# jh-jeong/ContraD

Hardware: AMD Instinct MI355X
Metric: discriminator-step images/sec (ContraD, SimCLR aug) (higher is better)
Workload: dtype f32; 1 GPU; SNDCGAN + ContraD D-step, CIFAR-10 32x32, global batch 512, simclr aug, nonsat loss, Adam(2e-4,(0.5,0.999)), random-init weights; global_batch=512, per_gpu_batch=512, parallelism=dp1, losses_finite=True, launch=hipGraph replay, rccl_ranks=1

## Files before the change

### contrad_amd/_lib.py

```python
import ctypes
import os
import re

_HERE = os.path.dirname(os.path.abspath(__file__))
LIB_PATH = os.environ.get('CONTRAD_HIP_LIB') or os.path.join(_HERE, 'csrc', 'libcontrad_hip.so')
HEADER_PATH = os.path.join(os.path.dirname(_HERE), 'include', 'contrad_hip.h')


class ConvDesc(ctypes.Structure):
    _fields_ = [(n, ctypes.c_int) for n in
                ('N', 'H', 'W', 'C', 'ldx', 'Ho', 'Wo', 'K', 'ldy', 'KH', 'KW', 'stride', 'pad', 'ldw')]


SN_MAX_LAYERS = 24
ADAM_MAX_TENSORS = 64
ADAM_CHUNK = 16384
AUG_NPARAM = 16


class SnLayer(ctypes.Structure):
    _fields_ = [('w', ctypes.c_void_p), ('u', ctypes.c_void_p), ('v', ctypes.c_void_p),
                ('u_snap', ctypes.c_void_p), ('v_snap', ctypes.c_void_p),
                ('wp', ctypes.c_void_p), ('gwp', ctypes.c_void_p), ('gw', ctypes.c_void_p),
                ('K', ctypes.c_int), ('C', ctypes.c_int), ('T', ctypes.c_int), ('ldw', ctypes.c_int),
# ... 43 lines not shown
                ('rowloss', ctypes.c_void_p), ('loss', ctypes.c_void_p), ('grad_scale', ctypes.c_void_p),
                ('dz', ctypes.c_void_p), ('workspace', ctypes.c_void_p), ('workspace_bytes', ctypes.c_longlong)]


class L2normProblem(ctypes.Structure):
    _fields_ = [('u', ctypes.c_void_p), ('z', ctypes.c_void_p), ('inv_norm', ctypes.c_void_p), ('dz', ctypes.c_void_p),
                ('du', ctypes.c_void_p), ('ldu', ctypes.c_int), ('R', ctypes.c_int), ('D', ctypes.c_int),
                ('accumulate', ctypes.c_int), ('zero_rows', ctypes.c_int)]


FILTER_MAX_JOBS = 16


class FilterJob(ctypes.Structure):
    _fields_ = [('wp', ctypes.c_void_p), ('U', ctypes.c_void_p), ('kind', ctypes.c_int), ('mode', ctypes.c_int),
                ('C', ctypes.c_int), ('K', ctypes.c_int), ('ldw', ctypes.c_int)]


class FilterBatch(ctypes.Structure):
    _fields_ = [('n', ctypes.c_int), ('jobs', FilterJob * FILTER_MAX_JOBS),
                ('block_start', ctypes.c_int * (FILTER_MAX_JOBS + 1))]


_CTYPES = {
    'int': ctypes.c_int,
    'float': ctypes.c_float,
    'double': ctypes.c_double,
    'long long': ctypes.c_longlong,
    'contrad_stream_t': ctypes.c_void_p,
    'void': None,
}


def _map_type(t):
    t = t.strip()
    if t.endswith('*'):
        base = t[:-1].replace('const', '').strip()
        if base == 'contrad_conv_desc':
            return ctypes.POINTER(ConvDesc)
        if base == 'int':
            return ctypes.POINTER(ctypes.c_int)
        return ctypes.c_void_p
    t = t.replace('const', '').strip()
    return _CTYPES[t]


# ... 48 lines not shown
```

### contrad_amd/csrc/igemm.hip

```cpp
#include "common.h"
#include <stdlib.h>
#include <string.h>
#include <algorithm>
#include <utility>
#include "../../include/contrad_hip.h"

namespace {

enum { MODE_FWD = 0, MODE_DGRAD = 1, MODE_WGRAD = 2 };
#ifndef IGEMM_BK
#define IGEMM_BK 16
#endif
constexpr int BK = IGEMM_BK;
#ifndef IGEMM_MIN_WAVES
#define IGEMM_MIN_WAVES 4
#endif
constexpr int NTHREADS = 256;

struct IgemmArgs {
  const float* A;
  const float* B;
  float* C;
  const float* bias;
  const float* addend;
  const float* act_ref;
  float* bias_ws;
  contrad_conv_desc d;
  float slope, gain;
  int M, Ncol, Kg;
  int tiles_m, tiles_n;
  int P;
  int ptiles_per_split;
  int ny;
  int cgroup;
  int cbal;
  int cb_reps[4], cb_start[5];
  int dsplits;
  long long slab_elems;
  int px_pixels;
  short win_h0[16], win_w0[16], win_hc[16], win_wc[16];
  int win_tile0[17];
  int nwin;
  unsigned char px_order[256];
  int pixmajor;
  int px_full;
  int st_nt;
};

constexpr long long NT_STORE_BYTES = 256ll << 20;
inline int st_nt_for(long long rows, int ld) {
#if defined(LEAN_ST_NT)
  if (LEAN_ST_NT >= 0) return LEAN_ST_NT;
#endif
  return rows * (long long)ld * (long long)sizeof(float) >= NT_STORE_BYTES ? 1 : 0;
}

__device__ __forceinline__ float4 ld4(const float* p) { return *reinterpret_cast<const float4*>(p); }
__device__ __forceinline__ float4 zero4() { return make_float4(0.f, 0.f, 0.f, 0.f); }

template <int MODE, int BM, int BN, bool VEC>
__global__ __launch_bounds__(NTHREADS, 2) void igemm_kernel(const IgemmArgs p) {
  extern __shared__ __attribute__((aligned(16))) float smem[];
  constexpr bool A_KCONTIG = (MODE != MODE_WGRAD);
  constexpr bool B_KCONTIG = (MODE == MODE_DGRAD);
  constexpr int LDA = BM + (A_KCONTIG ? 1 : 4);
  constexpr int LDB = BN + (B_KCONTIG ? 1 : 4);
  constexpr int A_SZ = BK * LDA, B_SZ = BK * LDB;
  constexpr int PA = BM * BK / 1024, PB = BN * BK / 1024;
  constexpr int KQ = BK / 4;
// ... 526 lines not shown
            p.C[off + c] = v;
          }
        }
      }
  } else {
#pragma unroll
    for (int i = 0; i < TM; ++i)
#pragma unroll
      for (int r = 0; r < 16; ++r) {
        const int m = m0 + wm * WM + i * 32 + (r & 3) + 8 * (r >> 2) + 4 * lhi;
        if (m >= M) continue;
#pragma unroll
        for (int j = 0; j < TN; ++j) {
          const int c = n0 + wn * WN + j * 32 + l31;
          if (c < Ncol) {
            float v = acc[i][j][r];
            if constexpr (MODE == MODE_FWD) {
              if (p.bias) v += p.bias[c];
              v = (v > 0.f) ? v : v * p.slope;
              v *= p.gain;
              if (p.addend) v += p.addend[(size_t)m * d.ldy + c];
              p.C[(size_t)m * d.ldy + c] = v;
            } else {
              p.C[((size_t)blockIdx.y * M + m) * Ncol + c] = v;
            }
          }
        }
      }
    if constexpr (MODE == MODE_WGRAD && VEC) {
      if (p.bias_ws != nullptr && tile_m == 0) {
        float* red = smem;
        *reinterpret_cast<float4*>(red + b_r * BN + b_c4 * 4) = colacc;
        __syncthreads();
        if (tid < BN) {
          float sum = 0.f;
#pragma unroll
          for (int r = 0; r < B_RPP; ++r) sum += red[r * BN + tid];
          const int c = n0 + tid;
          if (c < Ncol) p.bias_ws[(size_t)blockIdx.y * Ncol + c] = sum;
        }
      }
    }
  }
}

__global__ void wgrad_reduce_kernel(const float* __restrict__ ws, float* __restrict__ out, int Kg, int Ncol,
                                    int ldw, int splits, const float* __restrict__ bias_ws,
                                    float* __restrict__ dbias, int R) {
  const long long total = (long long)Kg * Ncol;
  const long long nthreads = (long long)gridDim.x * blockDim.x;
  const long long t0 = (long long)blockIdx.x * blockDim.x + threadIdx.x;
  const int r = (int)(t0 % R);
  const long long g0 = t0 / R, gstride = nthreads / R;
  if (ldw == Ncol && (total & 3) == 0) {
    const long long n4 = total / 4;
    for (long long q0 = g0 - (g0 % (64 / R)); q0 < n4; q0 += gstride) {
      const long long q = q0 + (g0 % (64 / R));
      float4 s = make_float4(0.f, 0.f, 0.f, 0.f);
      if (q < n4) {
        int k = r;
        for (; k + 3 * R < splits; k += 4 * R) {
          const float4 v0 = *reinterpret_cast<const float4*>(ws + (long long)k * total + q * 4);
          const float4 v1 = *reinterpret_cast<const float4*>(ws + (long long)(k + R) * total + q * 4);
          const float4 v2 = *reinterpret_cast<const float4*>(ws + (long long)(k + 2 * R) * total + q * 4);
          const float4 v3 = *reinterpret_cast<const float4*>(ws + (long long)(k + 3 * R) * total + q * 4);
          s.x += (v0.x + v1.x) + (v2.x + v3.x); s.y += (v0.y + v1.y) + (v2.y + v3.y);
          s.z += (v0.z + v1.z) + (v2.z + v3.z); s.w += (v0.w + v1.w) + (v2.w + v3.w);
        }
        for (; k < splits; k += R) {
          const float4 v = *reinterpret_cast<const float4*>(ws + (long long)k * total + q * 4);
          s.x += v.x; s.y += v.y; s.z += v.z; s.w += v.w;
        }
      }
      for (int o = R >> 1; o > 0; o >>= 1) {
// ... 6 lines not shown
    for (long long e0 = g0 - (g0 % (64 / R)); e0 < total; e0 += gstride) {
      const long long e = e0 + (g0 % (64 / R));
      float s = 0.f;
      if (e < total)
        for (int k = r; k < splits; k += R) s += ws[(long long)k * total + e];
      for (int o = R >> 1; o > 0; o >>= 1) s += __shfl_xor(s, o, 64);
      if (r == 0 && e < total) {
        const int i = (int)(e / Ncol), c = (int)(e - (long long)i * Ncol);
        out[(size_t)i * ldw + c] = s;
      }
    }
  }
  if (dbias)
    for (long long c0 = g0 - (g0 % (64 / R)); c0 < Ncol; c0 += gstride) {
      const long long c = c0 + (g0 % (64 / R));
      float s = 0.f;
      if (c < Ncol)
        for (int k = r; k < splits; k += R) s += bias_ws[(long long)k * Ncol + c];
      for (int o = R >> 1; o > 0; o >>= 1) s += __shfl_xor(s, o, 64);
      if (r == 0 && c < Ncol) dbias[c] = s;
    }
}

template <int BM, int BN>
constexpr size_t smem_bytes(int mode) {
  const int lda = BM + ((mode != MODE_WGRAD) ? 1 : 4);
  const int ldb = BN + ((mode == MODE_DGRAD) ? 1 : 4);
  size_t main_loop = 2 * (size_t)(BK * lda + BK * ldb) * sizeof(float);
  size_t epi = (size_t)BM * sizeof(long long);
  return main_loop > epi ? main_loop : epi;
}

template <auto Kernel, class Args>
int launch_large_lds(dim3 grid, int threads, size_t lds_bytes, hipStream_t stream, const Args& a) {
  static bool attr_set_dev[64] = {};
  int dev_id = 0;
  (void)hipGetDevice(&dev_id);
  bool& attr_set = attr_set_dev[dev_id & 63];
  if (!attr_set) {
    hipError_t e = hipFuncSetAttribute(reinterpret_cast<const void*>(Kernel), hipFuncAttributeMaxDynamicSharedMemorySize, (int)lds_bytes);
    if (e != hipSuccess) return (int)e;
    attr_set = true;
  }
  hipLaunchKernelGGL(Kernel, grid, dim3(threads), lds_bytes, stream, a);
  CONTRAD_CHECK_LAUNCH();
  return 0;
// ... 612 lines not shown
                                    int ldx, const float* __restrict__ act_ref, float slope, float gain,
                                    float* __restrict__ dx) {
  const int c4n = C >> 2;
  const long long total = rows * c4n;
  const float g1 = gain, g0 = gain * slope;
  for (long long e = (long long)blockIdx.x * blockDim.x + threadIdx.x; e < total;
       e += (long long)gridDim.x * blockDim.x) {
    const long long m = e / c4n;
    const long long off = m * ldx + (e - m * c4n) * 4;
    float4 v = ld4(ws + off);
    for (int k = 1; k < splits; ++k) {
      const float4 u = ld4(ws + (long long)k * slab + off);
      v.x += u.x; v.y += u.y; v.z += u.z; v.w += u.w;
    }
    if (act_ref) {
      const float4 a = ld4(act_ref + off);
      v.x *= (a.x > 0.f) ? g1 : g0; v.y *= (a.y > 0.f) ? g1 : g0;
      v.z *= (a.z > 0.f) ? g1 : g0; v.w *= (a.w > 0.f) ? g1 : g0;
    }
    *reinterpret_cast<float4*>(dx + off) = v;
  }
}

int launch_wgrad_reduce(const float* ws, float* dwp, int Kg, int K, int ldw, int slabs, const float* bias_ws, float* dbias,
                        hipStream_t stream) {
  const long long total = (long long)Kg * K;
  int R = 1;
  while (R < 64 && R * 2 <= slabs && (total / 4) * R < 65536) R <<= 1;
  const long long blocks = std::max(1ll, std::min(2048ll, ((total / 4) * R + 255) / 256));
  hipLaunchKernelGGL(wgrad_reduce_kernel, dim3((int)blocks), dim3(256), 0, stream, ws, dwp, Kg, K, ldw, slabs, bias_ws, dbias, R);
  CONTRAD_CHECK_LAUNCH();
  return 0;
}

template <int MODE>
int launch_wino_kind(int kind, const contrad_conv_desc* d, const float* in, const float* wp, const float* bias, const float* ref,
                     float* out, float slope, float gain, float* workspace, const contrad_filter_job* u, hipStream_t stream) {
  CONTRAD_ARG(aligned16(in, wp, workspace));
  const float* U = filter_fits(u, kind, MODE, d, wp) ? u->U : nullptr;
  const WinoFamily* f = wino_family(kind);
  CONTRAD_ARG(f && f->launch[MODE]);
  return f->launch[MODE](d, in, wp, bias, ref, out, slope, gain, workspace, stream, U);
}

enum Family {
  FAM_SCALAR = 0, FAM_GENERAL = 1, FAM_LEAN = 2, FAM_LEAN_SKIP = 3,
  FAM_WGRAD_C32 = 4, FAM_FWD_K1 = 5, FAM_CONV_C32 = 6,
  FAM_WINO = 7, FAM_WINO22 = 8, FAM_WINO44 = 9, FAM_WINO23 = 10, FAM_WINO44N = 11
};

inline const WinoFamily* wino_family_of(int family) { return wino_family(family == FAM_WINO44N ? FILTER_WINO44 : family); }

struct Route {
  int family;
  int filter_kind;
// ... 397 lines not shown
  const dim3 grid = mode == MODE_FWD ? fwd_setup(d, r.plan, &a) : mode == MODE_DGRAD ? dgrad_setup(d, r.plan, &a) : wgrad_setup(d, r.plan, &a);
  if (mode == MODE_FWD && !with_workspace) return grid.x;
  return (long long)grid.x * grid.y;
}

extern "C" int contrad_conv2d_tile_order(const contrad_conv_desc* d, int mode, unsigned char* out, int capacity) {
  if (check_desc(d) || (mode != MODE_FWD && mode != MODE_DGRAD) || !out || capacity <= 0) return -22;
  const Route r = conv_route(d, mode, true, 0);
  if (r.family != FAM_LEAN_SKIP || r.plan.pixmajor != 1 || r.plan.splits > 1) return 0;
  const int npix = mode == MODE_FWD ? d->Ho * d->Wo : cdiv(d->H, d->stride) * cdiv(d->W, d->stride);
  unsigned char order[256] = {};
  if (!pixel_table(d, mode, r.plan, npix, order)) return 0;
  const int nt = cdiv(d->N, r.plan.bm) * npix;
  if (nt > capacity) return -22;
  memcpy(out, order, (size_t)nt);
  return nt;
}

extern "C" long long contrad_conv2d_wgrad_workspace_bytes(const contrad_conv_desc* d) {
  if (check_desc(d)) return -22;
  return conv_route(d, MODE_WGRAD, true).workspace_bytes;
}

extern "C" int contrad_conv2d_wgrad(const contrad_conv_desc* d, const float* x, const float* gy,
                                    float* dwp, float* dbias, float* workspace, long long workspace_bytes,
                                    contrad_stream_t stream) {
  int rc = check_desc(d);
  if (rc) return rc;
  CONTRAD_ARG(x && gy && dwp && workspace);
  if (vec_ok(d, MODE_WGRAD)) CONTRAD_ARG(aligned16(x, gy, workspace));
  const Route r = conv_route(d, MODE_WGRAD, true);
  CONTRAD_ARG(workspace_bytes >= r.workspace_bytes);
  hipStream_t s = (hipStream_t)stream;
  const int Kg = d->KH * d->KW * d->C;
  switch (r.family) {
    case FAM_WINO: return launch_wgrad<WinoWgrad>(d, x, gy, dwp, dbias, workspace, s);
    case FAM_WINO22: return launch_wgrad<Wino22Wgrad>(d, x, gy, dwp, dbias, workspace, s);
    case FAM_WGRAD_C32: {
      const int blocks = wgrad_c32_blocks(d);
      float* bias_ws = dbias ? workspace + (size_t)blocks * Kg * d->K : nullptr;
      rc = launch_wgrad_c32(d, x, gy, workspace, bias_ws, s);
      return rc ? rc : launch_wgrad_reduce(workspace, dwp, Kg, d->K, d->ldw, blocks, bias_ws, dbias, s);
    }
    default: break;
  }
  const FwdPlan& p = r.plan;
  CONTRAD_ARG(dbias == nullptr || r.vec);
  CONTRAD_ARG((long long)d->N * d->Ho * d->Wo < (1ll << 31) - 4096);
  IgemmArgs a{};
  a.A = x; a.B = gy; a.C = workspace;
  a.bias_ws = dbias ? workspace + (size_t)p.splits * Kg * d->K : nullptr;
  const dim3 grid = wgrad_setup(d, p, &a);
  rc = dispatch<MODE_WGRAD>(a, p.bm, p.bn, r.vec, grid, s);
  return rc ? rc : launch_wgrad_reduce(workspace, dwp, Kg, d->K, d->ldw, p.splits, a.bias_ws, dbias, s);
}
```

### contrad_amd/csrc/igemm_lean.h

```cpp
#pragma once

#ifndef LEAN_DEEP
#define LEAN_DEEP 0
#endif
#ifndef LEAN_LD_NT
#define LEAN_LD_NT 0
#endif
#ifndef LEAN_ST_NT
#define LEAN_ST_NT -1
#endif
#ifndef LEAN_QPAD
#define LEAN_QPAD 8
#endif

constexpr unsigned LEAN_OOB = 0x80000000u;
constexpr unsigned LEAN_RANGE = 0x80000000u;
constexpr unsigned WB_TOP = 2u, WB_BOT = 4u, WB_LEFT = 8u, WB_RIGHT = 16u;

__device__ __forceinline__ float4 bload4(__amdgpu_buffer_rsrc_t r, unsigned voff, unsigned soff) {
  return __builtin_bit_cast(float4, __builtin_amdgcn_raw_buffer_load_b128(r, (int)voff, (int)soff, 0));
}

__device__ __forceinline__ __amdgpu_buffer_rsrc_t lean_rsrc(const float* base, bool on) {
  return __builtin_amdgcn_make_buffer_rsrc(const_cast<float*>(base), 0, on ? (int)LEAN_RANGE : 0, 0x00020000);
// ... 640 lines not shown
#pragma unroll
        for (int q = 0; q < EPI_G; ++q) {
#pragma unroll
          for (int jj = 0; jj < TN; ++jj) {
            const unsigned vo = offs[q] + colpart[jj];
            float v = acc[i][jj][r0 + q];
            if constexpr (MODE == MODE_DGRAD) {
              if (ref) v *= (rv[q][jj] > 0.f) ? g1 : g0;
            } else {
              v += bj[jj];
              v = (v > 0.f) ? v : v * p.slope;
              v *= p.gain;
              if (ref) v += rv[q][jj];
            }
            __builtin_amdgcn_raw_buffer_store_b32(__builtin_bit_cast(unsigned, v), rsC, (int)vo, 0, ST_AUX);
          }
        }
      }
    };
    if (st_nt && !(MODE == MODE_DGRAD && pl_dsplits > 1)) store_rows(std::true_type{}); else store_rows(std::false_type{});
  } else {
    const bool slab = (MODE == MODE_WGRAD) || p.ny > 1;
    const bool pxm = (MODE == MODE_FWD) && pl_pixmajor;
    const int pitch = pxm ? px_pitch : (slab ? Ncol : d.ldy);
    const size_t out_off = pxm ? (size_t)px_off : (slab ? (size_t)by * M * Ncol : (size_t)0) + (size_t)m0 * pitch;
    float* outp = p.C + out_off;
    const int rows_here = pxm ? px_rows : min(BM, M - m0);
    const __amdgpu_buffer_rsrc_t rsC = __builtin_amdgcn_make_buffer_rsrc(outp, 0, rows_here * pitch * 4, 0x00020000);
    const int wave_row = __builtin_amdgcn_readfirstlane(wm * WM);
    const float g1 = p.gain, g0 = p.gain * p.slope;
    const bool has_add = (MODE == MODE_FWD) && !slab && p.addend != nullptr;
    const __amdgpu_buffer_rsrc_t rsD = __builtin_amdgcn_make_buffer_rsrc(
        const_cast<float*>(has_add ? p.addend + out_off : outp), 0, has_add ? rows_here * pitch * 4 : 0, 0x00020000);
    unsigned lanepart[TN];
    float bj[TN];
#pragma unroll
    for (int j = 0; j < TN; ++j) {
      lanepart[j] = colpart[j] + (unsigned)(4 * lhi * pitch) * 4u;
      const int c = n0 + wn * WN + j * 32 + l31;
      bj[j] = (MODE == MODE_FWD && !slab && p.bias && c < Ncol) ? p.bias[c] : 0.f;
    }
    if constexpr (MODE == MODE_FWD) {
      constexpr int EPI_F = (BM * BN > 128 * 64) ? 4 : EPI_G;
      auto store_fwd = [&](auto nt_c) {
      constexpr int ST_AUX = decltype(nt_c)::value ? 2 : 0;
      constexpr int LD_AUX = (LEAN_LD_NT && decltype(nt_c)::value) ? 2 : 0;
#pragma unroll
// ... 129 lines not shown
```

### contrad_amd/csrc/wino_host.h

```cpp

constexpr int WINO_CUS = 256;

struct Sides { int cin, cout, ldi, ldo; };
inline Sides sides(const contrad_conv_desc* d, int mode) {
  if (mode == MODE_FWD) return {d->C, d->K, d->ldx, d->ldy};
  return {d->K, d->C, d->ldy, d->ldx};
}

inline bool fills_chip(long long items, long long min_items, int num, int den) {
  if (items < WINO_CUS) return items >= min_items;
  return cdivll(items, WINO_CUS) * WINO_CUS * den <= items * num;
}

inline int persistent_grid(int xcd_items) { return 8 * std::min(WINO_CUS / 8, xcd_items); }

template <class F>
int family_grid(const contrad_conv_desc* d, int mode) { return persistent_grid((int)F::items(F::args(d, mode), 8)); }

template <class F, int MODE>
int launch_family(const contrad_conv_desc* d, const float* in, const float* wp, const float* bias, const float* ref, float* out,
                  float slope, float gain, float* U, hipStream_t stream, const float* Uprep) {
  typename F::Args a = F::args(d, MODE);
  a.x = in; a.U = Uprep ? Uprep : U; a.y = out; a.bias = bias; a.ref = ref; a.slope = slope; a.gain = gain;
  const int quads = F::PHASES * (a.Cin / 4) * a.Cout;
// ... 265 lines not shown
  return nullptr;
}

inline long long filter_bytes(int kind, const contrad_conv_desc* d) {
  return (long long)wino_family(kind)->points * d->C * d->K * (long long)sizeof(float);
}

inline long long filter_threads(int kind, int mode, int C, int K) {
  const WinoFamily* f = wino_family(kind);
  if (!f || (mode != MODE_FWD && mode != MODE_DGRAD) || !f->launch[mode]) return 0;
  contrad_conv_desc d{};
  d.C = C; d.K = K;
  const Sides s = sides(&d, mode);
  return f->phases * (long long)(s.cin / 4) * s.cout;
}

inline bool filter_fits(const contrad_filter_job* u, int kind, int mode, const contrad_conv_desc* d, const float* wp) {
  return u && u->U && u->kind == kind && u->mode == mode && u->C == d->C && u->K == d->K && u->ldw == d->ldw && u->wp == wp &&
         ((uintptr_t)u->U & 15) == 0;
}

int launch_wgrad_reduce(const float* ws, float* dwp, int Kg, int K, int ldw, int slabs, const float* bias_ws, float* dbias,
                        hipStream_t stream);

inline int wgrad_qps(int chunks, int out_blocks) {
  const int splits = std::max(1, std::min(chunks, WINO_CUS / out_blocks));
  return cdiv(chunks, splits);
}

struct WinoWgrad {
  using Args = wino::WArgs;
  static constexpr int POINTS = 9;
  static constexpr auto kernel = wino::wino_wgrad_kernel;
  static constexpr size_t LDS_BYTES = wino::W_LDS_DWORDS * 4;
  static bool enabled() {
    static const bool on = contrad_dev_on("CONTRAD_WINO_WGRAD") && contrad_dev_on("CONTRAD_WINO");
    return on;
  }
  static bool ok(const contrad_conv_desc* d) {
    if (d->KH != 3 || d->KW != 3 || d->stride != 1 || d->pad != 1) return false;
    if (d->H < 4 || d->W < 4 || (d->H & (d->H - 1)) || (d->W & (d->W - 1))) return false;
    if ((d->C & 63) || (d->K & 63) || (d->ldx & 3) || (d->ldy & 3)) return false;
    const long long lim = 1ll << 31;
    if (2ll * d->H * d->W * std::max(d->ldx, d->ldy) * 4 >= lim) return false;
    return true;
  }
// ... 49 lines not shown
  }
  static int row_blocks(const Args& a) { return a.RBN; }
};

template <class G> int wgrad_splits(const typename G::Args& a) { return cdiv(a.Q, a.qps); }
template <class G> int wgrad_grid(const typename G::Args& a) { return G::row_blocks(a) * a.KB * wgrad_splits<G>(a); }

template <class G>
bool wgrad_planned(const contrad_conv_desc* d) {
  if (!G::enabled() || !G::ok(d)) return false;
  const typename G::Args a = G::args(d);
  const long long blocks = wgrad_grid<G>(a);
  static const int min_qps = contrad_dev_int("CONTRAD_WINO_MIN_QPS", 16);
  return a.qps >= min_qps && blocks * 10 >= WINO_CUS * 7 && blocks <= WINO_CUS;
}

template <class G>
long long wgrad_workspace_bytes(const contrad_conv_desc* d) {
  return (long long)wgrad_splits<G>(G::args(d)) * ((long long)G::POINTS * d->C + 1) * d->K * (long long)sizeof(float);
}

template <class G>
int launch_wgrad(const contrad_conv_desc* d, const float* x, const float* gy, float* dwp, float* dbias, float* workspace,
                 hipStream_t stream) {
  typename G::Args a = G::args(d);
  const int splits = wgrad_splits<G>(a);
  a.x = x; a.gy = gy; a.ws = workspace;
  a.bias_ws = dbias ? workspace + (size_t)splits * G::POINTS * d->C * d->K : nullptr;
  const int rc = launch_large_lds<G::kernel>(dim3(wgrad_grid<G>(a)), 512, G::LDS_BYTES, stream, a);
  return rc ? rc : launch_wgrad_reduce(workspace, dwp, G::POINTS * d->C, d->K, d->ldw, splits, a.bias_ws, dbias, stream);
}
```

### contrad_amd/models/gan/sndcgan.py

```python
import torch
import torch.nn as nn
import torch.distributed as dist

from ... import ops
from ...hostio import upload
from ... import autograd_ops as A
from .base import BaseDiscriminator, SNParams, TinyHead, _Act, make_projection

_D_CONVS = [(3, 64, 3, 1, 1), (64, 128, 4, 2, 1), (128, 128, 3, 1, 1), (128, 256, 4, 2, 1),
            (256, 256, 3, 1, 1), (256, 512, 4, 2, 1), (512, 512, 3, 1, 1)]
_SLOPE = 0.1


def _flat_views(total_sizes, device):
    offs, tot = [], 0
    for n in total_sizes:
        offs.append(tot)
        tot += ops.round_up(n, 4)
    buf = torch.empty(max(tot, 4), device=device, dtype=torch.float32)
    return buf, [buf[o:o + n] for o, n in zip(offs, total_sizes)]


class _DPlan(object):

# ... 124 lines not shown
        def _c(g, shape):
            if g is None:
                return torch.zeros(shape, device=dev, dtype=torch.float32)
            return g.contiguous()

        g_logits = _c(g_logits, (B, 1)).view(B, 1, 1, 1)
        g_proj = _c(g_proj, (B, dp)).view(B, 1, 1, dp)
        g_proj2 = _c(g_proj2, (B, dp)).view(B, 1, 1, dp)

        if need_params:
            gbuf, gv = _flat_views(plan.pack_sizes, dev)
            gwps = []
            for i, s in enumerate(specs[:7]):
                gwps.append(gv[i].view(s.T * s.C, s.K))
            gmerged = gv[7].view(plan.feat, 3 * dh)
            for j in range(3):
                gwps.append(gmerged[:, j * dh:(j + 1) * dh])
            gwps += [gv[8].view(dh, 4), gv[9].view(dh, dp), gv[10].view(dh, dp)]
            bsizes = [m.bias.numel() for m in plan.layers]
            bbuf, gbias = _flat_views(bsizes, dev)

        g_hidden = torch.empty((B, 1, 1, 3 * dh), device=dev, dtype=torch.float32)
        outs = [(g_logits, 10, 0), (g_proj, 11, 1), (g_proj2, 12, 2)]
        for g, li, j in outs:
            hs = hidden[..., j * dh:(j + 1) * dh]
            ops.conv2d_dgrad(g, wps[li], (B, 1, 1, dh), 1, 1, 1, 0, act_ref=hs, slope=_SLOPE, gain=1.0,
                             out=g_hidden[..., j * dh:(j + 1) * dh])
            if need_params:
                if g.shape[3] % 4 == 0:
                    ops.conv2d_wgrad(hs, g, 1, 1, 1, 0, out=gwps[li], dbias=gbias[li])
                else:
                    ops.conv2d_wgrad(hs, g, 1, 1, 1, 0, out=gwps[li])
                    ops.colstats(ops.as_rows(g), out=gbias[li].view(1, -1))
                exchange(gwps[li])
        if need_params:
            o7 = gbias[7].storage_offset()
            adjacent = all(gbias[7 + j].storage_offset() == o7 + j * dh for j in range(3))
            gb_hidden = bbuf[o7:o7 + 3 * dh] if adjacent else torch.empty(3 * dh, device=dev, dtype=torch.float32)
            ops.conv2d_wgrad(a6.view(B, 1, 1, plan.feat), g_hidden, 1, 1, 1, 0, out=gmerged, dbias=gb_hidden)
            exchange(gmerged)
            if not adjacent:
                for j in range(3):
                    gbias[7 + j].copy_(gb_hidden[j * dh:(j + 1) * dh])
        g = None
        if ctx.trunk_grad:
            lo = dh if ctx.sg_linear else 0
            fused = g_feats is None or g_feats.numel() == 0
            g = ops.conv2d_dgrad(g_hidden[..., lo:], ctx.merged[:, lo:], (B, 1, 1, plan.feat), 1, 1, 1, 0,
                                 act_ref=a6.view(B, 1, 1, plan.feat) if fused else None, slope=_SLOPE,
                                 gain=1.0).view(a6.shape)
            if not fused:
                g = g + g_feats.reshape(B, 512, plan.hb, plan.wb).permute(0, 2, 3, 1)
                g = (g * torch.where(a6 > 0, 1.0, _SLOPE)).contiguous()
            for i in range(6, 0, -1):
                ci, co, k, s, p = _D_CONVS[i]
                if need_params:
                    ops.conv2d_wgrad(acts[i - 1], g, k, k, s, p, out=gwps[i], dbias=gbias[i])
                    exchange(gwps[i])
                g = ops.conv2d_dgrad(g, wps[i], tuple(acts[i - 1].shape), k, k, s, p, act_ref=acts[i - 1],
                                     slope=_SLOPE, gain=1.0, filters=ctx.filters)
            if need_params:
                ops.rgb_conv_wgrad(images, g, 3, 2.0, -1.0, gwps[0], gbias[0])
                exchange(gwps[0])
        d_images = None
        if need_images and g is not None:
            d_images = ops.rgb_conv_dgrad(g, wps[0], None, 3, 3, act=0, out_scale=2.0, out_shift=0.0)

        grads = [None] * (2 * n)
        if need_params:
            if g is None:
                for i in range(7):
                    gwps[i].zero_(); gbias[i].zero_()
                    exchange(gwps[i])
            if comm is not None:
                exchange(bbuf)
                comm.wait()
            wsizes = [s.K * s.C * s.T for s in specs]
            gwbuf, gws = _flat_views(wsizes, dev)
            offs, scr_n = ops.sn_scratch_floats(specs)
            scratch = torch.empty(scr_n, device=dev, dtype=torch.float32)
            ops.sn_weight_grad(specs, wps, ldws, gwps, gws, scratch, offs, ctx.sigma, ctx.u_snaps, ctx.v_snaps)
            for i in range(n):
                grads[2 * i] = gws[i].view(ctx.param_shapes[2 * i])
                grads[2 * i + 1] = gbias[i]
        return (None, d_images, None, None, None) + tuple(grads)


class D_SNDCGAN(BaseDiscriminator):

    def __init__(self, image_size, ndf=64, n_classes=1, normalize=False, disable_sn=False, mlp_linear=True,
                 d_hidden=512, d_project=128):
        super().__init__()
# ... 235 lines not shown
```

### contrad_amd/ops.py

```python
import ctypes
import os

import torch

from ._lib import ConvDesc, ContrastProblem, FilterBatch, FilterJob, FILTER_MAX_JOBS, L2normProblem, lib


def _p(t):
    return ctypes.c_void_p(t.data_ptr()) if t is not None else ctypes.c_void_p(0)


_raw_stream = getattr(torch._C, '_cuda_getCurrentRawStream', None)


def _stream_handle():
    if _raw_stream is not None:
        return _raw_stream(torch.cuda.current_device())
    return torch.cuda.current_stream().cuda_stream


def _stream():
    return ctypes.c_void_p(_stream_handle())


def _chk(t, name):
    if t is None:
        return
    if not t.is_cuda or t.dtype != torch.float32:
# ... 77 lines not shown
    PROFILE.append((kname, flops, e0, e1, shape, int(blocks), executed))


def make_desc(N, H, W, C, K, KH, KW, stride, pad, ldx, ldy, ldw):
    return ConvDesc(N, H, W, C, ldx, out_size(H, KH, stride, pad), out_size(W, KW, stride, pad), K, ldy,
                    KH, KW, stride, pad, ldw)


def pack_weight(w):
    K, C, KH, KW = w.shape
    ldw = round_up(K, 4)
    wp = w.new_zeros(KH * KW * C, ldw)
    wp[:, :K] = w.permute(2, 3, 1, 0).reshape(KH * KW * C, K)
    return wp


def unpack_weight(wp, K, C, KH, KW):
    return wp[:, :K].reshape(KH, KW, C, K).permute(3, 2, 0, 1).contiguous()


FILTER_PREP = os.environ.get('CONTRAD_DEV_FILTER_PREP', '1') != '0'
CONTRAST_PAIR = os.environ.get('CONTRAD_DEV_CONTRAST_PAIR', '1') != '0'
BN_FUSED = os.environ.get('CONTRAD_DEV_BN_FUSED', '1') != '0'


def filter_kind(d, mode):
    nb = ctypes.c_longlong(0)
    kind = lib().raw('contrad_conv2d_filter_kind')(ctypes.byref(d), mode, ctypes.byref(nb))
    if kind < 0:
        raise RuntimeError('contrad_hip: bad conv descriptor (%d)' % kind)
    return kind, nb.value


def fwd_desc(x_shape, wp, K, KH, KW, stride, pad):
    N, H, W, C = x_shape
    return make_desc(N, H, W, C, K, KH, KW, stride, pad, C, K, wp.stride(0))


def dgrad_desc(x_shape, wp, K, KH, KW, stride, pad):
    return fwd_desc(x_shape, wp, K, KH, KW, stride, pad)


class PreparedFilters(object):

    def __init__(self):
        self.jobs = {}
# ... 146 lines not shown
    def __init__(self, owner_dict):
        self.mine = owner_dict

    def __enter__(self):
        global _ws_cache
        self.saved, _ws_cache = _ws_cache, self.mine
        return self

    def __exit__(self, *exc):
        global _ws_cache
        _ws_cache = self.saved
        return False


def _workspace(nbytes, device):
    key = (device.index, _stream_handle())
    buf = _ws_cache.get(key)
    if buf is None or buf.numel() * 4 < nbytes:
        buf = torch.empty((max(nbytes, 1) + 3) // 4, device=device, dtype=torch.float32)
        _ws_cache[key] = buf
    return buf


def conv2d_wgrad(x, gy, KH, KW, stride, pad, ldw=None, out=None, dbias=None):
    _chk(x, 'x'); _chk(gy, 'gy')
    N, H, W, C = x.shape
    K = gy.shape[3]
    if out is None:
        ldw = ldw or round_up(K, 4)
        out = torch.zeros((KH * KW * C, ldw), device=x.device, dtype=torch.float32)
    _chk(out, 'out')
    d = make_desc(N, H, W, C, K, KH, KW, stride, pad, _ld(x), _ld(gy), out.stride(0))
    nbytes = lib().raw('contrad_conv2d_wgrad_workspace_bytes')(ctypes.byref(d))
    if nbytes < 0:
        raise RuntimeError('contrad_hip: bad conv descriptor (%d)' % nbytes)
    ws = _workspace(nbytes, x.device)
    _conv_call(2, d, 'contrad_conv2d_wgrad', ctypes.byref(d), _p(x), _p(gy), _p(out), _p(dbias), _p(ws),
               ctypes.c_longlong(ws.numel() * 4), _stream())
    return out


def l2norm_fwd(u):
    _chk(u, 'u')
    R, D = u.shape
    z = torch.empty((R, D), device=u.device, dtype=torch.float32)
    inv = torch.empty((R,), device=u.device, dtype=torch.float32)
    lib().call('contrad_l2norm_fwd', _p(u), _ld(u), _p(z), _p(inv), R, D, 1e-12, _stream())
    return z, inv


def l2norm_bwd(dz, z, inv, out=None, accumulate=False):
    R, D = z.shape
    if out is None:
        out = torch.empty((R, D), device=z.device, dtype=torch.float32)
    lib().call('contrad_l2norm_bwd', _p(dz), _p(z), _p(inv), _p(out), _ld(out), R, D, int(accumulate), _stream())
# ... 837 lines not shown
```

### include/contrad_hip.h

```cpp
#ifndef CONTRAD_HIP_H
#define CONTRAD_HIP_H

#ifdef __cplusplus
extern "C" {
#endif

typedef void* contrad_stream_t;

int contrad_abi_version(void);

typedef struct {
  int N, H, W, C;
  int ldx;
  int Ho, Wo, K;
  int ldy;
  int KH, KW;
  int stride, pad;
  int ldw;
} contrad_conv_desc;

int contrad_conv2d_fwd(const contrad_conv_desc* d, const float* x, const float* wp, const float* bias,
                       float* y, float slope, float gain, float* workspace, long long workspace_bytes,
                       contrad_stream_t stream);
int contrad_conv2d_fwd_add(const contrad_conv_desc* d, const float* x, const float* wp, const float* bias,
// ... 32 lines not shown
} contrad_filter_job;
typedef struct {
  int n;
  contrad_filter_job jobs[CONTRAD_FILTER_MAX_JOBS];
  int block_start[CONTRAD_FILTER_MAX_JOBS + 1];
} contrad_filter_batch;
int contrad_conv2d_filter_kind(const contrad_conv_desc* d, int mode, long long* bytes);
int contrad_conv2d_filter_prep(const contrad_filter_batch* b, contrad_stream_t stream);
int contrad_conv2d_fwd_add_u(const contrad_conv_desc* d, const float* x, const float* wp, const float* bias,
                             const float* addend, float* y, float slope, float gain, float* workspace,
                             long long workspace_bytes, const contrad_filter_job* u, contrad_stream_t stream);
int contrad_conv2d_dgrad_ws_u(const contrad_conv_desc* d, const float* gy, const float* wp, float* dx,
                              const float* act_ref, float slope, float gain, float* workspace,
                              long long workspace_bytes, const contrad_filter_job* u, contrad_stream_t stream);

long long contrad_conv2d_wgrad_workspace_bytes(const contrad_conv_desc* d);
int contrad_conv2d_tile(const contrad_conv_desc* d, int mode, int* bm, int* bn);
int contrad_conv2d_path(const contrad_conv_desc* d, int mode);
double contrad_conv2d_executed_fraction(const contrad_conv_desc* d, int mode);
long long contrad_conv2d_grid_blocks(const contrad_conv_desc* d, int mode, int with_workspace);
int contrad_conv2d_tile_order(const contrad_conv_desc* d, int mode, unsigned char* out, int capacity);
int contrad_conv2d_wgrad(const contrad_conv_desc* d, const float* x, const float* gy, float* dwp,
                         float* dbias, float* workspace, long long workspace_bytes, contrad_stream_t stream);

long long contrad_contrast_workspace_bytes(int R, int D);
int contrad_contrast_fwd(const float* z, int R, int D, int N, int mode, float inv_temp, float* lse,
                         float* rowloss, float* loss, float* workspace, long long workspace_bytes,
                         contrad_stream_t stream);
int contrad_contrast_bwd(const float* z, const float* lse, int R, int D, int N, int mode, float inv_temp,
                         const float* grad_scale, float* dz, float* workspace, long long workspace_bytes,
                         contrad_stream_t stream);
int contrad_l2norm_fwd(const float* u, int ldu, float* z, float* inv_norm, int R, int D, float eps,
                       contrad_stream_t stream);
int contrad_l2norm_bwd(const float* dz, const float* z, const float* inv_norm, float* du, int ldu, int R,
                       int D, int accumulate, contrad_stream_t stream);

#define CONTRAD_CONTRAST_MAX_PROBLEMS 2
typedef struct {
  const float* z;
  int R, D, N, mode;
  float inv_temp;
  float* lse;
  float* rowloss;
  float* loss;
  const float* grad_scale;
  float* dz;
// ... 219 lines not shown
```

Measured before the change: 47250 images/sec.

## Defer weight-gradient split reductions into one batched reduce launch

Weight-gradient kernels now write their split-K partial slabs into a shared arena and return a reduce job instead of launching a reduce kernel each. All deferred jobs are then reduced in a single batched kernel at the end of the backward pass. When there is only one split, the igemm wgrad writes directly into the destination with the weight leading dimension, so that path skips the reduction. The aim is fewer small kernel launches and less slab traffic, at the cost of a larger arena that stays live across the whole backward pass and some changed ordering of the bias copy.

```diff
diff --git a/contrad_amd/_lib.py b/contrad_amd/_lib.py
--- a/contrad_amd/_lib.py
+++ b/contrad_amd/_lib.py
@@ -89,6 +89,20 @@
                 ('block_start', ctypes.c_int * (FILTER_MAX_JOBS + 1))]
 
 
+WGRAD_MAX_JOBS = 16
+
+
+class WgradJob(ctypes.Structure):
+    _fields_ = [('ws', ctypes.c_void_p), ('bias_ws', ctypes.c_void_p), ('dwp', ctypes.c_void_p), ('dbias', ctypes.c_void_p),
+                ('Kg', ctypes.c_int), ('K', ctypes.c_int), ('ldw', ctypes.c_int), ('slabs', ctypes.c_int),
+                ('R', ctypes.c_int), ('blocks', ctypes.c_int), ('direct', ctypes.c_int)]
+
+
+class WgradBatch(ctypes.Structure):
+    _fields_ = [('n', ctypes.c_int), ('jobs', WgradJob * WGRAD_MAX_JOBS),
+                ('block_start', ctypes.c_int * (WGRAD_MAX_JOBS + 1))]
+
+
 _CTYPES = {
     'int': ctypes.c_int,
     'float': ctypes.c_float,
diff --git a/contrad_amd/csrc/igemm.hip b/contrad_amd/csrc/igemm.hip
--- a/contrad_amd/csrc/igemm.hip
+++ b/contrad_amd/csrc/igemm.hip
@@ -45,6 +45,7 @@
   int pixmajor;
   int px_full;
   int st_nt;
+  int wg_direct;
 };
 
 constexpr long long NT_STORE_BYTES = 256ll << 20;
@@ -617,7 +618,7 @@
               if (p.addend) v += p.addend[(size_t)m * d.ldy + c];
               p.C[(size_t)m * d.ldy + c] = v;
             } else {
-              p.C[((size_t)blockIdx.y * M + m) * Ncol + c] = v;
+              p.C[((size_t)blockIdx.y * M + m) * (p.wg_direct ? d.ldw : Ncol) + c] = v;
             }
           }
         }
@@ -639,12 +640,12 @@
   }
 }
 
-__global__ void wgrad_reduce_kernel(const float* __restrict__ ws, float* __restrict__ out, int Kg, int Ncol,
-                                    int ldw, int splits, const float* __restrict__ bias_ws,
-                                    float* __restrict__ dbias, int R) {
+__device__ __forceinline__ void wgrad_reduce_body(const float* __restrict__ ws, float* __restrict__ out, int Kg, int Ncol,
+                                                  int ldw, int splits, const float* __restrict__ bias_ws,
+                                                  float* __restrict__ dbias, int R, int bid, int nblk) {
   const long long total = (long long)Kg * Ncol;
-  const long long nthreads = (long long)gridDim.x * blockDim.x;
-  const long long t0 = (long long)blockIdx.x * blockDim.x + threadIdx.x;
+  const long long nthreads = (long long)nblk * blockDim.x;
+  const long long t0 = (long long)bid * blockDim.x + threadIdx.x;
   const int r = (int)(t0 % R);
   const long long g0 = t0 / R, gstride = nthreads / R;
   if (ldw == Ncol && (total & 3) == 0) {
@@ -697,6 +698,20 @@
     }
 }
 
+__global__ void wgrad_reduce_kernel(const float* __restrict__ ws, float* __restrict__ out, int Kg, int Ncol,
+                                    int ldw, int splits, const float* __restrict__ bias_ws,
+                                    float* __restrict__ dbias, int R) {
+  wgrad_reduce_body(ws, out, Kg, Ncol, ldw, splits, bias_ws, dbias, R, (int)blockIdx.x, (int)gridDim.x);
+}
+
+__global__ void wgrad_reduce_batch_kernel(const contrad_wgrad_batch b) {
+  int j = 0;
+  while (j + 1 < b.n && (int)blockIdx.x >= b.block_start[j + 1]) ++j;
+  const contrad_wgrad_job& q = b.jobs[j];
+  wgrad_reduce_body(q.ws, q.dwp, q.Kg, q.K, q.ldw, q.slabs, q.bias_ws, q.dbias, q.R, (int)blockIdx.x - b.block_start[j],
+                    q.blocks);
+}
+
 template <int BM, int BN>
 constexpr size_t smem_bytes(int mode) {
   const int lda = BM + ((mode != MODE_WGRAD) ? 1 : 4);
@@ -1355,15 +1370,36 @@
   }
 }
 
-int launch_wgrad_reduce(const float* ws, float* dwp, int Kg, int K, int ldw, int slabs, const float* bias_ws, float* dbias,
-                        hipStream_t stream) {
+contrad_wgrad_job wgrad_job(const float* ws, float* dwp, int Kg, int K, int ldw, int slabs, const float* bias_ws, float* dbias) {
+  contrad_wgrad_job q{};
+  q.ws = ws; q.bias_ws = bias_ws; q.dwp = dwp; q.dbias = dbias;
+  q.Kg = Kg; q.K = K; q.ldw = ldw; q.slabs = slabs;
   const long long total = (long long)Kg * K;
   int R = 1;
   while (R < 64 && R * 2 <= slabs && (total / 4) * R < 65536) R <<= 1;
-  const long long blocks = std::max(1ll, std::min(2048ll, ((total / 4) * R + 255) / 256));
-  hipLaunchKernelGGL(wgrad_reduce_kernel, dim3((int)blocks), dim3(256), 0, stream, ws, dwp, Kg, K, ldw, slabs, bias_ws, dbias, R);
+  q.R = R;
+  q.blocks = (int)std::max(1ll, std::min(2048ll, ((total / 4) * R + 255) / 256));
+  return q;
+}
+
+contrad_wgrad_job wgrad_job_direct(float* dwp, int K, int ldw, const float* bias_ws, float* dbias) {
+  contrad_wgrad_job q = wgrad_job(nullptr, dwp, 0, K, ldw, 1, bias_ws, dbias);
+  q.blocks = dbias ? cdiv(K, 256) : 0;
+  q.direct = 1;
+  return q;
+}
+
+int launch_wgrad_job(const contrad_wgrad_job& q, hipStream_t stream) {
+  if (q.blocks == 0) return 0;
+  hipLaunchKernelGGL(wgrad_reduce_kernel, dim3(q.blocks), dim3(256), 0, stream, q.ws, q.dwp, q.Kg, q.K, q.ldw, q.slabs, q.bias_ws,
+                     q.dbias, q.R);
   CONTRAD_CHECK_LAUNCH();
   return 0;
+}
+
+int launch_wgrad_reduce(const float* ws, float* dwp, int Kg, int K, int ldw, int slabs, const float* bias_ws, float* dbias,
+                        hipStream_t stream) {
+  return launch_wgrad_job(wgrad_job(ws, dwp, Kg, K, ldw, slabs, bias_ws, dbias), stream);
 }
 
 template <int MODE>
@@ -1807,25 +1843,33 @@
   return conv_route(d, MODE_WGRAD, true).workspace_bytes;
 }
 
-extern "C" int contrad_conv2d_wgrad(const contrad_conv_desc* d, const float* x, const float* gy,
-                                    float* dwp, float* dbias, float* workspace, long long workspace_bytes,
-                                    contrad_stream_t stream) {
+namespace {
+int wgrad_main(const contrad_conv_desc* d, const float* x, const float* gy, float* dwp, float* dbias, float* workspace,
+               long long workspace_bytes, int force_wino, contrad_wgrad_job* job, hipStream_t s) {
   int rc = check_desc(d);
   if (rc) return rc;
-  CONTRAD_ARG(x && gy && dwp && workspace);
+  CONTRAD_ARG(x && gy && dwp && workspace && job);
+  if (force_wino) {
+    CONTRAD_ARG(aligned16(x, gy, workspace));
+    if (Wino22Wgrad::ok(d)) {
+      CONTRAD_ARG(workspace_bytes >= wgrad_workspace_bytes<Wino22Wgrad>(d));
+      return launch_wgrad<Wino22Wgrad>(d, x, gy, dwp, dbias, workspace, s, job);
+    }
+    CONTRAD_ARG(WinoWgrad::ok(d) && workspace_bytes >= wgrad_workspace_bytes<WinoWgrad>(d));
+    return launch_wgrad<WinoWgrad>(d, x, gy, dwp, dbias, workspace, s, job);
+  }
   if (vec_ok(d, MODE_WGRAD)) CONTRAD_ARG(aligned16(x, gy, workspace));
   const Route r = conv_route(d, MODE_WGRAD, true);
   CONTRAD_ARG(workspace_bytes >= r.workspace_bytes);
-  hipStream_t s = (hipStream_t)stream;
   const int Kg = d->KH * d->KW * d->C;
   switch (r.family) {
-    case FAM_WINO: return launch_wgrad<WinoWgrad>(d, x, gy, dwp, dbias, workspace, s);
-    case FAM_WINO22: return launch_wgrad<Wino22Wgrad>(d, x, gy, dwp, dbias, workspace, s);
+    case FAM_WINO: return launch_wgrad<WinoWgrad>(d, x, gy, dwp, dbias, workspace, s, job);
+    case FAM_WINO22: return launch_wgrad<Wino22Wgrad>(d, x, gy, dwp, dbias, workspace, s, job);
     case FAM_WGRAD_C32: {
       const int blocks = wgrad_c32_blocks(d);
       float* bias_ws = dbias ? workspace + (size_t)blocks * Kg * d->K : nullptr;
-      rc = launch_wgrad_c32(d, x, gy, workspace, bias_ws, s);
-      return rc ? rc : launch_wgrad_reduce(workspace, dwp, Kg, d->K, d->ldw, blocks, bias_ws, dbias, s);
+      *job = wgrad_job(workspace, dwp, Kg, d->K, d->ldw, blocks, bias_ws, dbias);
+      return launch_wgrad_c32(d, x, gy, workspace, bias_ws, s);
     }
     default: break;
   }
@@ -1833,9 +1877,47 @@
   CONTRAD_ARG(dbias == nullptr || r.vec);
   CONTRAD_ARG((long long)d->N * d->Ho * d->Wo < (1ll << 31) - 4096);
   IgemmArgs a{};
-  a.A = x; a.B = gy; a.C = workspace;
+  const bool direct = p.splits == 1;
+  a.A = x; a.B = gy; a.C = direct ? dwp : workspace;
+  a.wg_direct = direct ? 1 : 0;
   a.bias_ws = dbias ? workspace + (size_t)p.splits * Kg * d->K : nullptr;
   const dim3 grid = wgrad_setup(d, p, &a);
-  rc = dispatch<MODE_WGRAD>(a, p.bm, p.bn, r.vec, grid, s);
-  return rc ? rc : launch_wgrad_reduce(workspace, dwp, Kg, d->K, d->ldw, p.splits, a.bias_ws, dbias, s);
-}
+  *job = direct ? wgrad_job_direct(dwp, d->K, d->ldw, a.bias_ws, dbias)
+                : wgrad_job(workspace, dwp, Kg, d->K, d->ldw, p.splits, a.bias_ws, dbias);
+  return dispatch<MODE_WGRAD>(a, p.bm, p.bn, r.vec, grid, s);
+}
+}
+
+extern "C" int contrad_conv2d_wgrad(const contrad_conv_desc* d, const float* x, const float* gy,
+                                    float* dwp, float* dbias, float* workspace, long long workspace_bytes,
+                                    contrad_stream_t stream) {
+  contrad_wgrad_job q{};
+  const int rc = wgrad_main(d, x, gy, dwp, dbias, workspace, workspace_bytes, 0, &q, (hipStream_t)stream);
+  return rc ? rc : launch_wgrad_job(q, (hipStream_t)stream);
+}
+
+extern "C" int contrad_conv2d_wgrad_slabs(const contrad_conv_desc* d, const float* x, const float* gy, float* dwp, float* dbias,
+                                          float* workspace, long long workspace_bytes, int force_wino, contrad_wgrad_job* job,
+                                          contrad_stream_t stream) {
+  return wgrad_main(d, x, gy, dwp, dbias, workspace, workspace_bytes, force_wino, job, (hipStream_t)stream);
+}
+
+extern "C" int contrad_wgrad_reduce_batch(const contrad_wgrad_batch* b, contrad_stream_t stream) {
+  CONTRAD_ARG(b && b->n >= 0 && b->n <= CONTRAD_WGRAD_MAX_JOBS);
+  contrad_wgrad_batch k = *b;
+  long long blocks = 0;
+  for (int j = 0; j < k.n; ++j) {
+    const contrad_wgrad_job& q = k.jobs[j];
+    CONTRAD_ARG(q.dwp && q.K > 0 && q.ldw >= q.K && q.slabs >= 1 && q.Kg >= 0 && q.blocks >= 0 && q.blocks <= 2048);
+    CONTRAD_ARG(q.R >= 1 && q.R <= 64 && (q.R & (q.R - 1)) == 0 && (q.Kg == 0 || (q.ws && q.blocks > 0)));
+    CONTRAD_ARG(q.dbias == nullptr || q.bias_ws != nullptr);
+    CONTRAD_ARG((((uintptr_t)q.ws | (uintptr_t)q.dwp) & 15) == 0 || q.ldw != q.K || (((long long)q.Kg * q.K) & 3));
+    k.block_start[j] = (int)blocks;
+    blocks += q.blocks;
+  }
+  for (int j = k.n; j <= CONTRAD_WGRAD_MAX_JOBS; ++j) k.block_start[j] = (int)blocks;
+  if (blocks == 0) return 0;
+  hipLaunchKernelGGL(wgrad_reduce_batch_kernel, dim3((unsigned)blocks), dim3(256), 0, (hipStream_t)stream, k);
+  CONTRAD_CHECK_LAUNCH();
+  return 0;
+}
diff --git a/contrad_amd/csrc/igemm_lean.h b/contrad_amd/csrc/igemm_lean.h
--- a/contrad_amd/csrc/igemm_lean.h
+++ b/contrad_amd/csrc/igemm_lean.h
@@ -686,7 +686,8 @@
   } else {
     const bool slab = (MODE == MODE_WGRAD) || p.ny > 1;
     const bool pxm = (MODE == MODE_FWD) && pl_pixmajor;
-    const int pitch = pxm ? px_pitch : (slab ? Ncol : d.ldy);
+    const bool wg_direct = (MODE == MODE_WGRAD) && p.wg_direct;
+    const int pitch = pxm ? px_pitch : (slab ? (wg_direct ? d.ldw : Ncol) : d.ldy);
     const size_t out_off = pxm ? (size_t)px_off : (slab ? (size_t)by * M * Ncol : (size_t)0) + (size_t)m0 * pitch;
     float* outp = p.C + out_off;
     const int rows_here = pxm ? px_rows : min(BM, M - m0);
diff --git a/contrad_amd/csrc/wino_host.h b/contrad_amd/csrc/wino_host.h
--- a/contrad_amd/csrc/wino_host.h
+++ b/contrad_amd/csrc/wino_host.h
@@ -311,6 +311,7 @@
 
 int launch_wgrad_reduce(const float* ws, float* dwp, int Kg, int K, int ldw, int slabs, const float* bias_ws, float* dbias,
                         hipStream_t stream);
+contrad_wgrad_job wgrad_job(const float* ws, float* dwp, int Kg, int K, int ldw, int slabs, const float* bias_ws, float* dbias);
 
 inline int wgrad_qps(int chunks, int out_blocks) {
   const int splits = std::max(1, std::min(chunks, WINO_CUS / out_blocks));
@@ -406,11 +407,15 @@
 
 template <class G>
 int launch_wgrad(const contrad_conv_desc* d, const float* x, const float* gy, float* dwp, float* dbias, float* workspace,
-                 hipStream_t stream) {
+                 hipStream_t stream, contrad_wgrad_job* job = nullptr) {
   typename G::Args a = G::args(d);
   const int splits = wgrad_splits<G>(a);
   a.x = x; a.gy = gy; a.ws = workspace;
   a.bias_ws = dbias ? workspace + (size_t)splits * G::POINTS * d->C * d->K : nullptr;
   const int rc = launch_large_lds<G::kernel>(dim3(wgrad_grid<G>(a)), 512, G::LDS_BYTES, stream, a);
+  if (job) {
+    *job = wgrad_job(workspace, dwp, G::POINTS * d->C, d->K, d->ldw, splits, a.bias_ws, dbias);
+    return rc;
+  }
   return rc ? rc : launch_wgrad_reduce(workspace, dwp, G::POINTS * d->C, d->K, d->ldw, splits, a.bias_ws, dbias, stream);
 }
diff --git a/contrad_amd/models/gan/sndcgan.py b/contrad_amd/models/gan/sndcgan.py
--- a/contrad_amd/models/gan/sndcgan.py
+++ b/contrad_amd/models/gan/sndcgan.py
@@ -170,24 +170,33 @@
 
         g_hidden = torch.empty((B, 1, 1, 3 * dh), device=dev, dtype=torch.float32)
         outs = [(g_logits, 10, 0), (g_proj, 11, 1), (g_proj2, 12, 2)]
+        slabs = None
+        if need_params and comm is None and ops.SLAB_BATCH:
+            sizes = [ops.wgrad_bytes(hidden[..., j * dh:(j + 1) * dh], g, 1, 1, 1, 0, gwps[li].stride(0)) for g, li, j in outs]
+            sizes.append(ops.wgrad_bytes(a6.view(B, 1, 1, plan.feat), g_hidden, 1, 1, 1, 0, gmerged.stride(0)))
+            if ctx.trunk_grad:
+                for i in range(6, 0, -1):
+                    ci, co, k, s, p = _D_CONVS[i]
+                    sizes.append(ops.wgrad_bytes(acts[i - 1], acts[i], k, k, s, p, gwps[i].stride(0)))
+            slabs = ops.WgradSlabs(ops.WgradSlabs.arena_bytes(sizes), dev)
         for g, li, j in outs:
             hs = hidden[..., j * dh:(j + 1) * dh]
             ops.conv2d_dgrad(g, wps[li], (B, 1, 1, dh), 1, 1, 1, 0, act_ref=hs, slope=_SLOPE, gain=1.0,
                              out=g_hidden[..., j * dh:(j + 1) * dh])
             if need_params:
                 if g.shape[3] % 4 == 0:
-                    ops.conv2d_wgrad(hs, g, 1, 1, 1, 0, out=gwps[li], dbias=gbias[li])
+                    ops.conv2d_wgrad(hs, g, 1, 1, 1, 0, out=gwps[li], dbias=gbias[li], slabs=slabs)
                 else:
-                    ops.conv2d_wgrad(hs, g, 1, 1, 1, 0, out=gwps[li])
+                    ops.conv2d_wgrad(hs, g, 1, 1, 1, 0, out=gwps[li], slabs=slabs)
                     ops.colstats(ops.as_rows(g), out=gbias[li].view(1, -1))
                 exchange(gwps[li])
         if need_params:
             o7 = gbias[7].storage_offset()
             adjacent = all(gbias[7 + j].storage_offset() == o7 + j * dh for j in range(3))
             gb_hidden = bbuf[o7:o7 + 3 * dh] if adjacent else torch.empty(3 * dh, device=dev, dtype=torch.float32)
-            ops.conv2d_wgrad(a6.view(B, 1, 1, plan.feat), g_hidden, 1, 1, 1, 0, out=gmerged, dbias=gb_hidden)
+            ops.conv2d_wgrad(a6.view(B, 1, 1, plan.feat), g_hidden, 1, 1, 1, 0, out=gmerged, dbias=gb_hidden, slabs=slabs)
             exchange(gmerged)
-            if not adjacent:
+            if not adjacent and slabs is None:
                 for j in range(3):
                     gbias[7 + j].copy_(gb_hidden[j * dh:(j + 1) * dh])
         g = None
@@ -203,7 +212,7 @@
             for i in range(6, 0, -1):
                 ci, co, k, s, p = _D_CONVS[i]
                 if need_params:
-                    ops.conv2d_wgrad(acts[i - 1], g, k, k, s, p, out=gwps[i], dbias=gbias[i])
+                    ops.conv2d_wgrad(acts[i - 1], g, k, k, s, p, out=gwps[i], dbias=gbias[i], slabs=slabs)
                     exchange(gwps[i])
                 g = ops.conv2d_dgrad(g, wps[i], tuple(acts[i - 1].shape), k, k, s, p, act_ref=acts[i - 1],
                                      slope=_SLOPE, gain=1.0, filters=ctx.filters)
@@ -216,6 +225,11 @@
 
         grads = [None] * (2 * n)
         if need_params:
+            if slabs is not None:
+                slabs.reduce()
+                if not adjacent:
+                    for j in range(3):
+                        gbias[7 + j].copy_(gb_hidden[j * dh:(j + 1) * dh])
             if g is None:
                 for i in range(7):
                     gwps[i].zero_(); gbias[i].zero_()
diff --git a/contrad_amd/ops.py b/contrad_amd/ops.py
--- a/contrad_amd/ops.py
+++ b/contrad_amd/ops.py
@@ -3,7 +3,8 @@
 
 import torch
 
-from ._lib import ConvDesc, ContrastProblem, FilterBatch, FilterJob, FILTER_MAX_JOBS, L2normProblem, lib
+from ._lib import (ConvDesc, ContrastProblem, FilterBatch, FilterJob, FILTER_MAX_JOBS, L2normProblem, WgradBatch, WgradJob,
+                   WGRAD_MAX_JOBS, lib)
 
 
 def _p(t):
@@ -127,6 +128,7 @@
 FILTER_PREP = os.environ.get('CONTRAD_DEV_FILTER_PREP', '1') != '0'
 CONTRAST_PAIR = os.environ.get('CONTRAD_DEV_CONTRAST_PAIR', '1') != '0'
 BN_FUSED = os.environ.get('CONTRAD_DEV_BN_FUSED', '1') != '0'
+SLAB_BATCH = os.environ.get('CONTRAD_DEV_SLAB_BATCH', '1') != '0'
 
 
 def filter_kind(d, mode):
@@ -319,7 +321,49 @@
     return buf
 
 
-def conv2d_wgrad(x, gy, KH, KW, stride, pad, ldw=None, out=None, dbias=None):
+def wgrad_bytes(x, gy, KH, KW, stride, pad, ldw, wino=False):
+    N, H, W, C = x.shape
+    d = make_desc(N, H, W, C, gy.shape[3], KH, KW, stride, pad, _ld(x), _ld(gy), ldw)
+    if wino:
+        nbytes = lib().raw('contrad_conv2d_wino_workspace_bytes')(ctypes.byref(d), 2)
+    else:
+        nbytes = lib().raw('contrad_conv2d_wgrad_workspace_bytes')(ctypes.byref(d))
+    if nbytes < 0:
+        raise RuntimeError('contrad_hip: bad conv descriptor (%d)' % nbytes)
+    return nbytes
+
+
+class WgradSlabs(object):
+
+    def __init__(self, nbytes, device):
+        self.buf = torch.empty((max(nbytes, 1) + 3) // 4, device=device, dtype=torch.float32)
+        self.used = 0
+        self.jobs = []
+
+    def region(self, nbytes):
+        n = round_up(nbytes, 256) // 4
+        if self.used + n > self.buf.numel():
+            raise RuntimeError('contrad_hip: weight-gradient slab arena too small')
+        r = self.buf[self.used:self.used + n]
+        self.used += n
+        return r
+
+    @staticmethod
+    def arena_bytes(sizes):
+        return sum(round_up(b, 256) for b in sizes)
+
+    def reduce(self):
+        jobs, self.jobs = self.jobs, []
+        for start in range(0, len(jobs), WGRAD_MAX_JOBS):
+            b = WgradBatch()
+            chunk = jobs[start:start + WGRAD_MAX_JOBS]
+            b.n = len(chunk)
+            for i, j in enumerate(chunk):
+                b.jobs[i] = j
+            lib().call('contrad_wgrad_reduce_batch', ctypes.byref(b), _stream())
+
+
+def conv2d_wgrad(x, gy, KH, KW, stride, pad, ldw=None, out=None, dbias=None, slabs=None, wino=False):
     _chk(x, 'x'); _chk(gy, 'gy')
     N, H, W, C = x.shape
     K = gy.shape[3]
@@ -328,6 +372,14 @@
         out = torch.zeros((KH * KW * C, ldw), device=x.device, dtype=torch.float32)
     _chk(out, 'out')
     d = make_desc(N, H, W, C, K, KH, KW, stride, pad, _ld(x), _ld(gy), out.stride(0))
+    if slabs is not None:
+        nbytes = wgrad_bytes(x, gy, KH, KW, stride, pad, out.stride(0), wino)
+        ws = slabs.region(nbytes)
+        job = WgradJob()
+        _conv_call(2, d, 'contrad_conv2d_wgrad_slabs', ctypes.byref(d), _p(x), _p(gy), _p(out), _p(dbias), _p(ws),
+                   ctypes.c_longlong(nbytes), int(wino), ctypes.byref(job), _stream())
+        slabs.jobs.append(job)
+        return out
     nbytes = lib().raw('contrad_conv2d_wgrad_workspace_bytes')(ctypes.byref(d))
     if nbytes < 0:
         raise RuntimeError('contrad_hip: bad conv descriptor (%d)' % nbytes)
diff --git a/include/contrad_hip.h b/include/contrad_hip.h
--- a/include/contrad_hip.h
+++ b/include/contrad_hip.h
@@ -78,6 +78,25 @@
 int contrad_conv2d_tile_order(const contrad_conv_desc* d, int mode, unsigned char* out, int capacity);
 int contrad_conv2d_wgrad(const contrad_conv_desc* d, const float* x, const float* gy, float* dwp,
                          float* dbias, float* workspace, long long workspace_bytes, contrad_stream_t stream);
+#define CONTRAD_WGRAD_MAX_JOBS 16
+typedef struct {
+  const float* ws;
+  const float* bias_ws;
+  float* dwp;
+  float* dbias;
+  int Kg, K, ldw, slabs;
+  int R, blocks;
+  int direct;
+} contrad_wgrad_job;
+typedef struct {
+  int n;
+  contrad_wgrad_job jobs[CONTRAD_WGRAD_MAX_JOBS];
+  int block_start[CONTRAD_WGRAD_MAX_JOBS + 1];
+} contrad_wgrad_batch;
+int contrad_conv2d_wgrad_slabs(const contrad_conv_desc* d, const float* x, const float* gy, float* dwp, float* dbias,
+                               float* workspace, long long workspace_bytes, int force_wino, contrad_wgrad_job* job,
+                               contrad_stream_t stream);
+int contrad_wgrad_reduce_batch(const contrad_wgrad_batch* b, contrad_stream_t stream);
 
 long long contrad_contrast_workspace_bytes(int R, int D);
 int contrad_contrast_fwd(const float* z, int R, int D, int N, int mode, float inv_temp, float* lse,
```

Result: no change. 47420 images/sec, median of 6 (+0.4%).
